# culiver/VAR

Measured on AMD Instinct MI355X. Metric: 256x256 images/sec (CFG=1.5) VAR-d16, higher is better.
Workload: dtype f32

## Files before the change

### include/var_hip.h

```cpp
#ifndef VAR_HIP_H
#define VAR_HIP_H

#include <stdint.h>

#ifdef __cplusplus
extern "C" {
#endif

#define VARHIP_EINVAL (-1)

typedef void* varhip_stream_t;

const char* varhip_version(void);

#define VARHIP_EPI_NONE 0
#define VARHIP_EPI_GELU 1
#define VARHIP_EPI_RESID 2
int varhip_gemm_nt_f32(const float* A, int64_t lda, const float* W, int64_t ldw, const float* bias,
                       float* out, int64_t ldo, int M, int N, int K, int epi,
                       const float* resid, int64_t ldr, const float* gamma, int64_t ldg, int rows_per_group,
                       int bias_per_row, int batch, int64_t sA, int64_t sW, int64_t sO, varhip_stream_t stream);
int varhip_gemm_force_tile(int tile);
int varhip_gemm_qkv_force_tile(int tile);
int varhip_gemm_last_pick(void);
// ... 70 lines not shown
int varhip_rans_encode_host(const uint32_t* pairs, int64_t n, uint32_t* words_out, int64_t cap, int64_t* nwords_out);
int varhip_rans_decode_u32(const uint32_t* cum, int l, int V, const uint32_t* words, int64_t words_total, const int64_t* word_off,
                           const int64_t* nwords, uint32_t* state, int64_t* idx_out, int32_t* err_out, int B, varhip_stream_t stream);
int varhip_rans_decode_host(const uint32_t* cum, int l, int V, const uint32_t* words, int64_t words_total, const int64_t* word_off,
                            const int64_t* nwords, uint32_t* state, int64_t* idx_out, int32_t* err_out, int B);

int varhip_quant_accum_f32(const int64_t* idx, const float* codebook, const int32_t* tap_idx, const float* tap_w,
                           const float* phi_w, const float* phi_b, float ratio,
                           float* up, float* f_hat, int B, int pn, int P, int Cv, varhip_stream_t stream);

int varhip_quant_accum_h_f32(const float* h, const int32_t* tap_idx, const float* tap_w,
                             const float* phi_w, const float* phi_b, float ratio,
                             float* up, float* f_hat, int B, int pn, int P, int Cv, varhip_stream_t stream);

int varhip_gumbel_softmax_f32(const float* x, const float* noise, float* y, int64_t rows, int V, float mul, float tau, varhip_stream_t stream);

int varhip_next_map_f32(const float* f_hat, const float* word_w, const float* word_b, const float* lvl_pos,
                        float* x_out, float* pooled, int B, int P, int pq, int C, int Cv, varhip_stream_t stream);
int varhip_quant_last_route(void);

int varhip_lvl_pos_f32(const float* lvl_embed, const int64_t* lvl, const float* pos, float* out, int L, int C, varhip_stream_t stream);

int varhip_first_map_f32(const float* class_emb, const int64_t* labels, int num_classes, const float* pos_start,
                         const float* lvl_pos, float* cond, float* x_out, int B, int C, int first_l, varhip_stream_t stream);

int varhip_conv3x3_nhwc_f32(const float* in, const float* w, const float* bias, const float* resid, float* out,
                            int B, int H, int W, int Cin, int Cout, int up2, int out_mode, varhip_stream_t stream);

int varhip_upconv_pack_f32(const float* w, float* w_phase, int Cin, int Cout, varhip_stream_t stream);
int varhip_upconv_phase_f32(const float* in, const float* w_phase, const float* bias, float* out,
                            int B, int H, int W, int Cin, int Cout, varhip_stream_t stream);
int varhip_upconv_phase_gn_f32(const float* in, const float* w_phase, const float* bias, float* out, double* gn_part,
                               int B, int H, int W, int Cin, int Cout, varhip_stream_t stream);

int64_t varhip_gn_scratch_elems(int B, int HW, int C, int G);
int varhip_gn_stats_f32(const float* x, float* stats, double* scratch, int B, int HW, int C, int G, float eps, varhip_stream_t stream);
int varhip_gn_apply_f32(const float* x, const float* stats, const float* gamma, const float* beta, float* out,
                        int B, int HW, int C, int G, int silu, varhip_stream_t stream);

int varhip_gn_silu_conv_out_f32(const float* x, const float* stats, const float* gamma, const float* beta, const float* w, const float* bias,
                                float* out, int B, int H, int W, int Cin, int Cout, int G, int out_mode, varhip_stream_t stream);

int varhip_softmax_rows_f32(const float* x, float* out, int64_t rows, int n, float scale, varhip_stream_t stream);

int varhip_nchw_to_nhwc_f32(const float* in, float* out, int B, int C, int HW, varhip_stream_t stream);
int varhip_nhwc_to_nchw_f32(const float* in, float* out, int B, int C, int HW, varhip_stream_t stream);

int varhip_conv_gn_blocks(int H, int W, int Cout, int phase);
int varhip_conv3x3_gn_nhwc_f32(const float* in, const float* w, const float* bias, const float* resid, float* out, double* gn_part,
                               int B, int H, int W, int Cin, int Cout, int up2, varhip_stream_t stream);
int varhip_gn_stats_part_f32(const double* gn_part, float* stats, int B, int nblk, int HW, int C, int G, float eps, varhip_stream_t stream);
int varhip_conv3x3_wino_nhwc_f32(const float* in, const float* u, const float* bias, const float* resid, float* out, double* gn_part,
                                 int B, int H, int W, int Cin, int Cout, varhip_stream_t stream);
int varhip_conv3x3_s2_nhwc_f32(const float* in, const float* w, const float* bias, float* out,
                               int B, int H, int W, int Cin, int Cout, varhip_stream_t stream);
int varhip_conv3x3_s2_nhwc_f16(const void* in, const void* w, const float* bias, void* out, int B, int H, int W, int Cin, int Cout,
                               varhip_stream_t stream);
int varhip_conv3x3_s2_nhwc_bf16(const void* in, const void* w, const float* bias, void* out, int B, int H, int W, int Cin, int Cout,
                                varhip_stream_t stream);
int varhip_nchw_to_nhwc_pad_f32(const float* in, float* out, int B, int C, int HW, int Cpad, varhip_stream_t stream);
int varhip_area_pool_f32(const float* f, float* pooled, int B, int P, int pq, int Cv, varhip_stream_t stream);
int varhip_word_embed_f32(const float* pooled, const float* word_w, const float* word_b, const float* lvl_pos,
                          float* x_out, int B, int lq, int C, int Cv, varhip_stream_t stream);
int varhip_quant_residual_f32(const int64_t* idx, const float* codebook, const int32_t* tap_idx, const float* tap_w,
                              const float* phi_w, const float* phi_b, float ratio, float* up, float* f_hat, float* f_rest,
                              int B, int pn, int P, int Cv, varhip_stream_t stream);

int varhip_token_select_i64(const uint8_t* keep, const int64_t* gt, const int64_t* sampled, int64_t* out, int64_t n, varhip_stream_t stream);

int varhip_neighbor_table_f32(const float* codebook, int V, int D, int n, int32_t* nbr_idx, float* nbr_dist, varhip_stream_t stream);
int varhip_smooth_select_f32(const float* logits, const int64_t* gt, const int32_t* nbr_idx, const float* nbr_dist, int n,
                             int cand_count, int use_thr, float thr, float ratio, int B, int l, int V, double t_cfg,
                             int64_t* idx_out, float* maxval_out, float* distlp_out, float* cfg_out, varhip_stream_t stream);

int varhip_token_loglik_f32(const float* logits, const int64_t* gt, int64_t ld_gt, int images, int classes, int l, int V,
                            int with_uncond, float ca, float cb, float* out, int64_t ld_out_img, int64_t ld_out_cls, varhip_stream_t stream);

int varhip_code_dist_f32(const float* codebook, int V, int D, float* out, varhip_stream_t stream);
int varhip_token_score_f32(const float* logits, const int64_t* gt, int64_t ld_gt, int images, int classes, int l, int V,
                           int with_uncond, float ca, float cb, int mode, int param, float thr, const float* dist, int64_t ld_dist,
                           float* out, int64_t ld_out_img, int64_t ld_out_cls, varhip_stream_t stream);

int varhip_dist_profile_f32(const float* logits, const int64_t* gt, int64_t ld_gt, int images, int classes, int l, int V,
                            int with_uncond, float ca, float cb, const float* dist, int64_t ld_dist,
                            const float* edges, int nbins, float min_prob,
                            int64_t* mass_q, int64_t* count, int64_t ld_img, int64_t ld_cls, varhip_stream_t stream);

int varhip_class_mix_f32(const float* logits, const int64_t* gt, int64_t ld_gt, int images, int classes, int l, int V, int with_uncond,
                         float ca, float cb, const float* prior, int64_t ld_prior, float* entropy, int64_t ld_ent_img, int64_t ld_ent_cls,
                         int64_t* mix_q, int64_t* hcond_q, int32_t* nanflag, int64_t ld_acc, float* h_mix, float* h_cond, float* mi,
                         float* logp_mix, int64_t ld_out, varhip_stream_t stream);
int varhip_class_mix_finish_f32(const int64_t* mix_q, const int64_t* hcond_q, const int32_t* nanflag, int64_t ld_acc, const int64_t* gt,
                                int64_t ld_gt, int images, int l, int V, float* h_mix, float* h_cond, float* mi, float* logp_mix,
                                int64_t ld_out, varhip_stream_t stream);
int varhip_class_mix_host_f32(const float* logits, const int64_t* gt, int64_t ld_gt, int images, int classes, int l, int V, int with_uncond,
                              float ca, float cb, const float* prior, int64_t ld_prior, float* entropy, int64_t ld_ent_img, int64_t ld_ent_cls,
                              int64_t* mix_q, int64_t* hcond_q, int32_t* nanflag, int64_t ld_acc, float* h_mix, float* h_cond, float* mi,
                              float* logp_mix, int64_t ld_out);
int varhip_class_mix_finish_host_f32(const int64_t* mix_q, const int64_t* hcond_q, const int32_t* nanflag, int64_t ld_acc, const int64_t* gt,
                                     int64_t ld_gt, int images, int l, int V, float* h_mix, float* h_cond, float* mi, float* logp_mix,
                                     int64_t ld_out);

int varhip_attn_profile_f32(const float* q, const float* kcache, int B2, int l, int H, int curL, int Lmax, const int32_t* ends, int S1,
                            int pn, int radius, int64_t* share_sum, int64_t ld_row, int64_t ld_head, int32_t* nan_count,
                            int32_t* tokens, int64_t ld_tok_row, int64_t ld_tok_head, varhip_stream_t stream);
int varhip_attn_profile_host_f32(const float* q, const float* kcache, int B2, int l, int H, int curL, int Lmax, const int32_t* ends, int S1,
// ... 134 lines not shown
                            int B, int H, int W, int Cin, int Cout, varhip_stream_t stream);
int varhip_conv16_gn_fusable(int B, int H, int W, int Cin, int Cout);
int varhip_gnconv3x3_nhwc_f16(const void* in, const float* table, int silu,
                              const void* w, const float* bias, const void* resid, void* out, double* gn_part,
                              int B, int H, int W, int Cin, int Cout, varhip_stream_t stream);
int varhip_gn_scale_shift_f32(const float* stats, const float* gamma, const float* beta, float* table, int B, int C, int G, varhip_stream_t stream);
int varhip_conv16_force_tile(int wm);
int varhip_conv16_last_pick(void);
int varhip_gn_stats_f16(const void* x, float* stats, double* scratch, int B, int HW, int C, int G, float eps, varhip_stream_t stream);
int varhip_gn_apply_f16(const void* x, const float* stats, const float* gamma, const float* beta, void* out,
                        int B, int HW, int C, int G, int silu, varhip_stream_t stream);
int varhip_gn_silu_conv_out_f16(const void* x, const float* stats, const float* gamma, const float* beta, const void* w, const float* bias,
                                float* out, int B, int H, int W, int Cin, int Cout, int G, int out_mode, varhip_stream_t stream);
int varhip_cast_f32_to_f16(const float* in, void* out, int64_t n, varhip_stream_t stream);
int varhip_cast_f16_to_f32(const void* in, float* out, int64_t n, varhip_stream_t stream);

int varhip_gemm_nt_bf16(const void* A, int64_t lda, const void* W, int64_t ldw, const float* bias,
                       void* out, int64_t ldo, int out_f16, int M, int N, int K, int epi,
                       const void* resid, int64_t ldr, int resid_f16, const float* gamma, int64_t ldg, int rows_per_group,
                       int batch, int64_t sA, int64_t sW, int64_t sO, varhip_stream_t stream);
int varhip_gemm16_force_tile(int tile);
int varhip_gemm16_persistent(int on);
int varhip_gemm16_deep(int on);
int varhip_gemm16_last_pick(int i);
int varhip_gemm_qkv_bf16(const void* A, int64_t lda, const void* W, int64_t ldw, const float* bias, int M, int C, int K,
                        const float* scale_mul, float plain_scale, int l2norm,
                        void* q_out, void* kcache, void* vcache, int B2, int l, int H, int pos0, int Lmax, varhip_stream_t stream);
int varhip_attn_cached_bf16(const void* q, const void* kcache, const void* vcache, void* out,
                           int B2, int l, int H, int curL, int Lmax, varhip_stream_t stream);
int varhip_ln_modulate_bf16out(const float* x, const float* scale, int64_t ld_scale, const float* shift, int64_t ld_shift,
                              void* out, int M, int C, int rows_per_group, float eps, varhip_stream_t stream);
int varhip_adaln_block_bf16(float* x, float* x2, void* xn16, void* q16, void* att16, void* hid16, const float* ada, int64_t ld_ada,
                           const void* qkv_w16, const float* qkv_b, const float* scale_mul, float plain_scale, int l2norm,
                           const void* proj_w16, const float* proj_b, const void* fc1_w16, const float* fc1_b,
                           const void* fc2_w16, const float* fc2_b, void* kcache16, void* vcache16,
                           int B2, int l, int C, int H, int hidden, int pos0, int Lmax, float eps, varhip_stream_t stream);
int varhip_conv3x3_nhwc_bf16(const void* in, const void* w, const float* bias, const void* resid, void* out, double* gn_part,
                            int B, int H, int W, int Cin, int Cout, int out_mode, varhip_stream_t stream);
int varhip_upconv_phase_bf16(const void* in, const void* w_phase, const float* bias, void* out, double* gn_part,
                            int B, int H, int W, int Cin, int Cout, varhip_stream_t stream);
int varhip_gnconv3x3_nhwc_bf16(const void* in, const float* table, int silu,
                               const void* w, const float* bias, const void* resid, void* out, double* gn_part,
                               int B, int H, int W, int Cin, int Cout, varhip_stream_t stream);
int varhip_conv16_force_tile(int wm);
int varhip_gn_stats_bf16(const void* x, float* stats, double* scratch, int B, int HW, int C, int G, float eps, varhip_stream_t stream);
int varhip_gn_apply_bf16(const void* x, const float* stats, const float* gamma, const float* beta, void* out,
                        int B, int HW, int C, int G, int silu, varhip_stream_t stream);
int varhip_gn_silu_conv_out_bf16(const void* x, const float* stats, const float* gamma, const float* beta, const void* w, const float* bias,
                                 float* out, int B, int H, int W, int Cin, int Cout, int G, int out_mode, varhip_stream_t stream);
int varhip_cast_f32_to_bf16(const float* in, void* out, int64_t n, varhip_stream_t stream);
int varhip_cast_bf16_to_f32(const void* in, float* out, int64_t n, varhip_stream_t stream);


#define VARHIP_NFAM 17
int varhip_timing_enable(int on);
int varhip_timing_select(int family_mask);
int varhip_timing_reset(void);
int varhip_timing_read(double* ms, double* flops, double* bytes, int64_t* launches);
const char* varhip_timing_name(int family);

#ifdef __cplusplus
}
#endif
#endif
```

### var_amd/csrc/common.h

```cpp
#pragma once
#include <hip/hip_runtime.h>
#include <stdint.h>
#include <stdlib.h>
#include "../../include/var_hip.h"
#include "../../include/var_math.h"

typedef float f32x2 __attribute__((ext_vector_type(2)));
__device__ __forceinline__ f32x2 vh_exp_pair(f32x2 x) {
    const f32x2 xc = {__builtin_fminf(x[0], 88.0f), __builtin_fminf(x[1], 88.0f)};
    const f32x2 t = xc * 1.44269504088896341f;
    const f32x2 n = {__builtin_rintf(t[0]), __builtin_rintf(t[1])};
    f32x2 r = __builtin_elementwise_fma(n, (f32x2)(-0.693145751953125f), xc);
    r = __builtin_elementwise_fma(n, (f32x2)(-1.42860682030941723212e-6f), r);
    f32x2 q = (f32x2)(1.9875691500e-4f);
    q = __builtin_elementwise_fma(q, r, (f32x2)(1.3981999507e-3f));
    q = __builtin_elementwise_fma(q, r, (f32x2)(8.3334519073e-3f));
    q = __builtin_elementwise_fma(q, r, (f32x2)(4.1665795894e-2f));
    q = __builtin_elementwise_fma(q, r, (f32x2)(1.6666665459e-1f));
    q = __builtin_elementwise_fma(q, r, (f32x2)(5.0000001201e-1f));
    const f32x2 y = __builtin_elementwise_fma(q, r * r, r) + 1.0f;
    f32x2 o;
    o[0] = (x[0] > -87.0f) ? __builtin_ldexpf(y[0], (int)n[0]) : 0.0f;
    o[1] = (x[1] > -87.0f) ? __builtin_ldexpf(y[1], (int)n[1]) : 0.0f;
    return o;
}

__device__ __forceinline__ f32x2 vh_gelu_tanh_pair(f32x2 x) {
    const f32x2 x3 = (x * x) * x;
    const f32x2 u = (x + x3 * 0.044715f) * 0.7978845608028654f;
    const f32x2 d = vh_exp_pair(u * -2.0f) + 1.0f;
    return f32x2{x[0] / d[0], x[1] / d[1]};
}

typedef float f32x4 __attribute__((ext_vector_type(4)));
typedef float f32x16 __attribute__((ext_vector_type(16)));

#define VH_FAM_GEMM 0
#define VH_FAM_CONV 1
#define VH_FAM_ATTN 2
#define VH_FAM_SAMPLER 3
#define VH_FAM_LN 4
#define VH_FAM_QKV 5
#define VH_FAM_GN 6
#define VH_FAM_OTHER 7
#define VH_FAM_GEMM_SMALL 8
#define VH_FAM_CONV_SMALL 9
#define VH_FAM_GEMM16 10
#define VH_FAM_GEMM16_SMALL 11
#define VH_FAM_CONV16H 12
#define VH_FAM_CONV16_SMALL 13
#define VH_FAM_ATTN16 14
#define VH_FAM_CONV_WINO 15
#define VH_FAM_ATTN_PROFILE 16

int vh_timing_on(int fam);
void vh_timing_begin(int fam, hipStream_t s, double flops, double bytes);
void vh_timing_end(int fam, hipStream_t s);

struct VhScope {
    int fam; hipStream_t s; bool on;
    VhScope(int f, hipStream_t st, double flops, double bytes) : fam(f), s(st), on(vh_timing_on(f) != 0) { if (on) vh_timing_begin(fam, s, flops, bytes); }
    ~VhScope() { if (on) vh_timing_end(fam, s); }
};

__device__ __forceinline__ void vh_dma16_buf(__amdgpu_buffer_rsrc_t rsrc, uint32_t voff, uint32_t soff, uint32_t lds) {
    asm volatile("s_mov_b32 m0, %3\n\ts_nop 0\n\tbuffer_load_dwordx4 %0, %1, %2 offen lds"
                 : : "v"(voff), "s"(rsrc), "s"(__builtin_amdgcn_readfirstlane(soff)), "s"(__builtin_amdgcn_readfirstlane(lds)) : "memory", "m0");
}

void vh_quant_phi_accum(const float* up, const float* phi_w, const float* phi_b, float ratio, float* f_hat, int B, int P, int Cv, hipStream_t s);

int vh_attn_keysel_refused(const void* q, const void* kcache, const void* vcache, const void* out, int B2, int l, int H, int curL, int Lmax,
                           const int32_t* ends, int S1, const int32_t* keymask, int32_t* ends16);

static inline int vh_launch_status() {
    hipError_t e = hipGetLastError();
    return e == hipSuccess ? 0 : -(1000 + (int)e);
}

template <int CTRL> __device__ __forceinline__ float vh_mov_dpp(float v) {
    return __int_as_float(__builtin_amdgcn_mov_dpp(__float_as_int(v), CTRL, 0xF, 0xF, true));
}
__device__ __forceinline__ float vh_lane_xor4(float v) {
    const float up = vh_mov_dpp<0x104>(v), dn = vh_mov_dpp<0x114>(v);
    return (threadIdx.x & 4) ? dn : up;
}
__device__ __forceinline__ float vh_wave_sum(float p) {
    { const auto r = __builtin_amdgcn_permlane32_swap(__float_as_uint(p), __float_as_uint(p), false, false); p = __uint_as_float(r[0]) + __uint_as_float(r[1]); }
    { const auto r = __builtin_amdgcn_permlane16_swap(__float_as_uint(p), __float_as_uint(p), false, false); p = __uint_as_float(r[0]) + __uint_as_float(r[1]); }
    p = p + vh_mov_dpp<0x128>(p);
    p = p + vh_lane_xor4(p);
    p = p + vh_mov_dpp<0x4E>(p);
    p = p + vh_mov_dpp<0xB1>(p);
    return p;
}
__device__ __forceinline__ float vh_wave_max(float p) {
    { const auto r = __builtin_amdgcn_permlane32_swap(__float_as_uint(p), __float_as_uint(p), false, false); p = fmaxf(__uint_as_float(r[0]), __uint_as_float(r[1])); }
    { const auto r = __builtin_amdgcn_permlane16_swap(__float_as_uint(p), __float_as_uint(p), false, false); p = fmaxf(__uint_as_float(r[0]), __uint_as_float(r[1])); }
    p = fmaxf(p, vh_mov_dpp<0x128>(p));
    p = fmaxf(p, vh_lane_xor4(p));
    p = fmaxf(p, vh_mov_dpp<0x4E>(p));
    p = fmaxf(p, vh_mov_dpp<0xB1>(p));
    return p;
}
__device__ __forceinline__ float vh_block_sum256(float p, float* red) {
    p = vh_wave_sum(p);
    __syncthreads();
    if ((threadIdx.x & 63) == 0) red[threadIdx.x >> 6] = p;
    __syncthreads();
    return ((red[0] + red[1]) + red[2]) + red[3];
}
__device__ __forceinline__ float vh_block_max256(float p, float* red) {
    p = vh_wave_max(p);
    __syncthreads();
    if ((threadIdx.x & 63) == 0) red[threadIdx.x >> 6] = p;
    __syncthreads();
    return fmaxf(fmaxf(red[0], red[1]), fmaxf(red[2], red[3]));
}
```

### var_amd/csrc/gemm.hip

```cpp
#include "common.h"

struct GemmP {
    const float* A; const float* W; const float* bias; float* out; const float* resid; const float* gamma;
    int64_t lda, ldw, ldo, ldr, ldg, sA, sW, sO;
    int M, N, K, epi, rows_per_group, bias_per_row;
    int H, Wd, Cin, up2, out_mode, Hi, Wi;
    int tilesM, tilesN;
    int evec;
    const float* q_smul; float* q_out; float* q_kc; float* q_vc; float q_plain; int q_l2, q_l, q_pos0, q_Lmax;
    double* gn_part;
};

__global__ void __launch_bounds__(256) k_gemm_any(GemmP p) {
    const int lane = threadIdx.x & 63, wave = threadIdx.x >> 6, r = lane & 31, h = lane >> 5;
    const int tm = blockIdx.x / p.tilesN, tn = blockIdx.x - tm * p.tilesN, bz = blockIdx.z;
    const int m0 = tm * 64 + (wave >> 1) * 32, n0 = tn * 64 + (wave & 1) * 32;
    const int ma = m0 + r, nb = n0 + r;
    const float* a = p.A + (int64_t)bz * p.sA + (int64_t)(ma < p.M ? ma : 0) * p.lda;
    const float* w = p.W + (int64_t)bz * p.sW + (int64_t)(nb < p.N ? nb : 0) * p.ldw;
    float* Ob = p.out + (int64_t)bz * p.sO;
    f32x16 acc;
#pragma unroll
    for (int e = 0; e < 16; ++e) acc[e] = 0.f;
    for (int k0 = 0; k0 < p.K; k0 += 2) {
// ... 592 lines not shown
}
extern "C" int varhip_conv3x3_nhwc_f32(const float* in, const float* w, const float* bias, const float* resid, float* out,
                                       int B, int H, int W, int Cin, int Cout, int up2, int out_mode, varhip_stream_t stream) {
    return conv3x3_impl(in, w, bias, resid, out, nullptr, B, H, W, Cin, Cout, up2, out_mode, stream);
}
extern "C" int varhip_conv3x3_gn_nhwc_f32(const float* in, const float* w, const float* bias, const float* resid, float* out, double* gn_part,
                                          int B, int H, int W, int Cin, int Cout, int up2, varhip_stream_t stream) {
    if (!gn_part) return VARHIP_EINVAL;
    return conv3x3_impl(in, w, bias, resid, out, gn_part, B, H, W, Cin, Cout, up2, 0, stream);
}

extern "C" int varhip_conv3x3_s2_nhwc_f32(const float* in, const float* w, const float* bias, float* out,
                                          int B, int H, int W, int Cin, int Cout, varhip_stream_t stream) {
    if (B <= 0 || H <= 0 || W <= 0 || Cin <= 0 || Cout <= 0 || (Cin & 31) || !bias) return VARHIP_EINVAL;
    if ((int64_t)B * H * W >= (1ll << 31)) return VARHIP_EINVAL;
    GemmP p{};
    p.A = in; p.W = w; p.bias = bias; p.out = out;
    p.ldw = 9ll * Cin; p.ldo = Cout; p.ldr = Cout;
    p.M = B * H * W; p.N = Cout; p.K = 9 * Cin; p.epi = VARHIP_EPI_NONE; p.rows_per_group = 1;
    p.H = H; p.Wd = W; p.Cin = Cin; p.up2 = 3; p.out_mode = 0; p.Hi = 2 * H; p.Wi = 2 * W;
    p.evec = !((Cout & 3) || ((uintptr_t)out & 15) || ((uintptr_t)bias & 15));
    const double npix = (double)B * H * W;
    VhScope scope(conv_family(3, Cout), (hipStream_t)stream, 2.0 * npix * Cout * 9.0 * Cin, 4.0 * (npix * 4 * Cin + npix * Cout + 9.0 * Cin * Cout));
    hipStream_t s = (hipStream_t)stream;
    return launch_conv(p, 1, s);
}

__global__ void k_upconv_pack(const float* __restrict__ w, float* __restrict__ wp, int Cout, int Cin) {
    const int64_t i = (int64_t)blockIdx.x * blockDim.x + threadIdx.x;
    const int64_t tot = (int64_t)16 * Cout * Cin;
    if (i >= tot) return;
    const int ci = (int)(i % Cin); int64_t t = i / Cin; const int b = (int)(t & 1), a = (int)((t >> 1) & 1); t >>= 2;
    const int co = (int)(t % Cout), ph = (int)(t / Cout), py = ph >> 1, px = ph & 1;
    const int ky0 = (py == 0) ? (a == 0 ? 0 : 1) : (a == 0 ? 0 : 2), ky1 = (py == 0) ? (a == 0 ? 0 : 2) : (a == 0 ? 1 : 2);
    const int kx0 = (px == 0) ? (b == 0 ? 0 : 1) : (b == 0 ? 0 : 2), kx1 = (px == 0) ? (b == 0 ? 0 : 2) : (b == 0 ? 1 : 2);
    float s = 0.f;
    for (int ky = ky0; ky <= ky1; ++ky)
        for (int kx = kx0; kx <= kx1; ++kx) s = s + w[(((int64_t)co * 3 + ky) * 3 + kx) * Cin + ci];
    wp[i] = s;
}
extern "C" int varhip_upconv_pack_f32(const float* w, float* w_phase, int Cin, int Cout, varhip_stream_t stream) {
    if (Cin <= 0 || Cout <= 0) return VARHIP_EINVAL;
    const int64_t tot = (int64_t)16 * Cout * Cin;
    VhScope scope(VH_FAM_OTHER, (hipStream_t)stream, 0, 4.0 * tot);
    hipLaunchKernelGGL(k_upconv_pack, dim3((unsigned)((tot + 255) / 256)), dim3(256), 0, (hipStream_t)stream, w, w_phase, Cout, Cin);
    return vh_launch_status();
}

static int upconv_phase_impl(const float* in, const float* w_phase, const float* bias, float* out, double* gn_part,
                             int B, int H, int W, int Cin, int Cout, varhip_stream_t stream) {
    if (B <= 0 || H <= 0 || W <= 0 || (H & 1) || (W & 1) || Cin <= 0 || Cout <= 0 || (Cin & 31) || !bias) return VARHIP_EINVAL;
    if (gn_part && !varhip_conv_gn_blocks(H, W, Cout, 1)) return VARHIP_EINVAL;
    if ((int64_t)B * H * W >= (1ll << 31)) return VARHIP_EINVAL;
    GemmP p{};
    p.A = in; p.W = w_phase; p.bias = bias; p.out = out; p.resid = nullptr; p.gamma = nullptr;
    p.ldw = 4ll * Cin; p.ldo = Cout; p.ldr = Cout; p.sW = (int64_t)Cout * 4 * Cin;
    p.M = B * (H / 2) * (W / 2); p.N = Cout; p.K = 4 * Cin; p.epi = VARHIP_EPI_NONE; p.rows_per_group = 1;
    p.H = H / 2; p.Wd = W / 2; p.Cin = Cin; p.up2 = 2; p.out_mode = 0; p.Hi = H / 2; p.Wi = W / 2;
    p.evec = !((Cout & 3) || ((uintptr_t)out & 15) || ((uintptr_t)bias & 15));
    if (gn_part && !p.evec) return VARHIP_EINVAL;
    p.gn_part = gn_part;
    const double npix = (double)B * H * W;
    VhScope scope(conv_family(2, Cout), (hipStream_t)stream, 2.0 * npix * Cout * 4.0 * Cin, 4.0 * (npix * Cin / 4.0 + npix * Cout + 16.0 * Cin * Cout));
    hipStream_t s = (hipStream_t)stream;
    return launch_conv(p, 4, s);
}
extern "C" int varhip_upconv_phase_f32(const float* in, const float* w_phase, const float* bias, float* out,
                                       int B, int H, int W, int Cin, int Cout, varhip_stream_t stream) {
    return upconv_phase_impl(in, w_phase, bias, out, nullptr, B, H, W, Cin, Cout, stream);
}
extern "C" int varhip_upconv_phase_gn_f32(const float* in, const float* w_phase, const float* bias, float* out, double* gn_part,
                                          int B, int H, int W, int Cin, int Cout, varhip_stream_t stream) {
    if (!gn_part) return VARHIP_EINVAL;
    return upconv_phase_impl(in, w_phase, bias, out, gn_part, B, H, W, Cin, Cout, stream);
}
```

### var_amd/csrc/timing.hip

```cpp
#include "common.h"
#include <mutex>
#include <vector>

namespace {
struct Rec { hipEvent_t a, b; int fam; };
std::mutex g_mu;
int g_on = 0;
int g_mask = ~0;
std::vector<Rec> g_pool;
size_t g_used = 0;
double g_ms[VARHIP_NFAM], g_flops[VARHIP_NFAM], g_bytes[VARHIP_NFAM];
int64_t g_n[VARHIP_NFAM];
const size_t kMaxRecs = 1 << 15;

void drain_locked() {
    for (size_t i = 0; i < g_used; ++i) {
        float ms = 0.f;
        if (hipEventSynchronize(g_pool[i].b) == hipSuccess && hipEventElapsedTime(&ms, g_pool[i].a, g_pool[i].b) == hipSuccess)
            g_ms[g_pool[i].fam] += ms;
    }
    g_used = 0;
}
}

// ... 14 lines not shown

void vh_timing_end(int fam, hipStream_t s) {
    std::lock_guard<std::mutex> lk(g_mu);
    (void)fam;
    if (g_used < g_pool.size()) { (void)hipEventRecord(g_pool[g_used].b, s); ++g_used; }
}

int vh_g_force_tile16 = -1;
int vh_g_gemm16_persist = [] { const char* e = getenv("VARHIP_GEMM16_PERSIST"); return e ? (atoi(e) != 0) : 1; }();
int vh_g_gemm16_deep = [] { const char* e = getenv("VARHIP_GEMM16_DEEP"); return e ? (atoi(e) != 0) : 1; }();
int vh_g_conv16_force_wm = 0;
int vh_g_gemm16_last_pick[2] = {0, 0};
int vh_g_gemm16_nlaunch = 0;
int vh_g_conv16_last_pick = -1;
int vh_g_attn16_last_waves = 0;

extern "C" {

int varhip_gemm16_force_tile(int tile) { vh_g_force_tile16 = (tile >= 0 && tile <= 3) ? tile : -1; return 0; }
int varhip_gemm16_persistent(int on) { vh_g_gemm16_persist = on ? 1 : 0; return 0; }
int varhip_gemm16_deep(int on) { vh_g_gemm16_deep = on ? 1 : 0; return 0; }
int varhip_gemm16_last_pick(int i) { return (i == 0 || i == 1) ? vh_g_gemm16_last_pick[i] : 0; }
int varhip_conv16_force_tile(int wm) { vh_g_conv16_force_wm = (wm == 2 || wm == 4 || wm == 8) ? wm : 0; return 0; }
int varhip_conv16_last_pick(void) { return vh_g_conv16_last_pick; }
int varhip_attn16_last_waves(void) { return vh_g_attn16_last_waves; }

const char* varhip_version(void) { return "var_hip 0.1.0 gfx950"; }

int varhip_timing_enable(int on) { std::lock_guard<std::mutex> lk(g_mu); g_on = on ? 1 : 0; return 0; }
int varhip_timing_select(int family_mask) { std::lock_guard<std::mutex> lk(g_mu); g_mask = family_mask; return 0; }

int varhip_timing_reset(void) {
    std::lock_guard<std::mutex> lk(g_mu);
    drain_locked();
    for (int i = 0; i < VARHIP_NFAM; ++i) { g_ms[i] = g_flops[i] = g_bytes[i] = 0.0; g_n[i] = 0; }
    return 0;
}

int varhip_timing_read(double* ms, double* flops, double* bytes, int64_t* launches) {
    std::lock_guard<std::mutex> lk(g_mu);
    drain_locked();
    for (int i = 0; i < VARHIP_NFAM; ++i) {
        if (ms) ms[i] = g_ms[i];
        if (flops) flops[i] = g_flops[i];
        if (bytes) bytes[i] = g_bytes[i];
        if (launches) launches[i] = g_n[i];
    }
    return VARHIP_NFAM;
}

const char* varhip_timing_name(int f) {
    static const char* names[VARHIP_NFAM] = {"gemm", "conv3x3", "attn", "sampler", "ln", "qkv_prep", "gn", "other", "gemm_small", "conv_small",
                                               "gemm16", "gemm16_small", "conv16h", "conv16_small", "attn16",
                                               "conv_wino", "attn_profile"};
    return (f >= 0 && f < VARHIP_NFAM) ? names[f] : "?";
}

}
```

### var_amd/csrc/winograd.hip

```cpp
#include <cstdlib>
#include <type_traits>

#include "common.h"

namespace {

constexpr int WG_PT = 18;
constexpr int WG_NDMA = 21;
constexpr int WG_STAGE = WG_NDMA * 16 * 64;
constexpr int WG_ZSTR = 20;
constexpr int WG_LDS = 2 * WG_STAGE;
static_assert(8 * 64 * WG_ZSTR * 4 <= WG_LDS, "epilogue exchange must fit in the K-loop stages");

struct WinoP {
    const float* in; const float* u; const float* bias; const float* resid; float* out; double* gn_part;
    int H, W, Cin, Cout, ncg, pw, ppi;
};

__device__ __forceinline__ void wg_wait_dma_barrier() { asm volatile("s_waitcnt vmcnt(8)\n\ts_barrier" ::: "memory"); }

constexpr int WG_KO_NOEPI = 1, WG_KO_NOGN = 2, WG_KO_NORES = 4, WG_KO_NOBTDB = 8;

__device__ __forceinline__ int wg_swz(int pix) { return (pix >> 1) & 3; }

// ... 134 lines not shown

    float* zb = smem;
    const int nblk = (H * W) >> 7;
#pragma unroll
    for (int cb = 0; cb < 2; ++cb) {
#pragma unroll
        for (int tb = 0; tb < 4; ++tb) {
            const f32x4 m0 = acc[0][tb][cb], m1 = acc[1][tb][cb], m2 = acc[2][tb][cb], m3 = acc[3][tb][cb];
            const f32x4 z0 = (m0 + m1) + m2, z1 = (m1 - m2) - m3;
            const int t = tb * 16 + r16;
            *(f32x4*)(zb + ((wave * 2 + 0) * 64 + t) * WG_ZSTR + 4 * kq) = z0;
            *(f32x4*)(zb + ((wave * 2 + 1) * 64 + t) * WG_ZSTR + 4 * kq) = z1;
        }
        __syncthreads();
        f32x4 z[4][2];
#pragma unroll
        for (int i = 0; i < 4; ++i)
#pragma unroll
            for (int bb = 0; bb < 2; ++bb) z[i][bb] = *(const f32x4*)(zb + ((i * 2 + bb) * 64 + et) * WG_ZSTR + 4 * eq);
        const int co = c0 + cb * 16 + 4 * eq;
        double gs[4] = {0.0, 0.0, 0.0, 0.0}, gq[4] = {0.0, 0.0, 0.0, 0.0};
#pragma unroll
        for (int a = 0; a < 2; ++a)
#pragma unroll
            for (int bb = 0; bb < 2; ++bb) {
                const f32x4 yv = a == 0 ? (z[0][bb] + z[1][bb]) + z[2][bb] : (z[1][bb] - z[2][bb]) - z[3][bb];
                f32x4 v = yv + b4[cb];
                const int64_t o = obase + ((int64_t)a * W + bb) * Cout + cb * 16;
                if constexpr (RES) v = rs[cb][a][bb] + v;
                *(f32x4*)(p.out + o) = v;
                if constexpr (GN) {
#pragma unroll
                    for (int e = 0; e < 4; ++e) { const double d = (double)v[e]; gs[e] += d; gq[e] += d * d; }
                }
            }
        if constexpr (GN) {
            const double t8[8] = {gs[0], gq[0], gs[1], gq[1], gs[2], gq[2], gs[3], gq[3]};
            const bool h4 = lane & 16, h3 = lane & 8, h2 = lane & 4;
            double r4[4], r2[2], r1;
#pragma unroll
            for (int i = 0; i < 4; ++i) r4[i] = (h4 ? t8[4 + i] : t8[i]) + __shfl_xor(h4 ? t8[i] : t8[4 + i], 16, 64);
#pragma unroll
            for (int i = 0; i < 2; ++i) r2[i] = (h3 ? r4[2 + i] : r4[i]) + __shfl_xor(h3 ? r4[i] : r4[2 + i], 8, 64);
            r1 = (h2 ? r2[1] : r2[0]) + __shfl_xor(h2 ? r2[0] : r2[1], 4, 64);
            r1 += __shfl_xor(r1, 2, 64);
            r1 += __shfl_xor(r1, 1, 64);
            if ((lane & 3) == 0)
                p.gn_part[(((int64_t)b * nblk + 2 * pi + (lane >> 5)) * Cout + co) * 2 + ((lane >> 2) & 7)] = r1;
        }
        if (cb == 0) __syncthreads();
    }
}

}

extern "C" int varhip_conv3x3_wino_nhwc_f32(const float* in, const float* u, const float* bias, const float* resid, float* out, double* gn_part,
                                            int B, int H, int W, int Cin, int Cout, varhip_stream_t stream) {
    if (!in || !u || !bias || !out || B <= 0 || H <= 0 || W <= 0 || Cin <= 0 || Cout <= 0) return VARHIP_EINVAL;
    if ((H & 15) || (W & 15) || (Cin & 31) || (Cout & 31)) return VARHIP_EINVAL;
    if ((((uintptr_t)in | (uintptr_t)u | (uintptr_t)bias | (uintptr_t)out | (uintptr_t)resid) & 15)) return VARHIP_EINVAL;
    if ((int64_t)H * W * Cin * 4 >= (1ll << 31) || 64ll * Cin * Cout >= (1ll << 31) || (int64_t)B * H * W >= (1ll << 31))
        return VARHIP_EINVAL;
    const int ppi = (H / 16) * (W / 16), ncg = Cout / 32;
    const int64_t nwg = (int64_t)B * ppi * ncg;
    if (nwg >= (1ll << 31)) return VARHIP_EINVAL;
    WinoP p{};
    p.in = in; p.u = u; p.bias = bias; p.resid = resid; p.out = out; p.gn_part = gn_part;
    p.H = H; p.W = W; p.Cin = Cin; p.Cout = Cout; p.ncg = ncg; p.pw = W / 16; p.ppi = ppi;
    const double npix = (double)B * H * W;
    VhScope scope(VH_FAM_CONV_WINO, (hipStream_t)stream, 2.0 * (npix / 4.0) * 16.0 * Cin * Cout,
                  4.0 * (npix * Cin + npix * Cout * (resid ? 2.0 : 1.0) + 16.0 * Cin * Cout));
    static const int dbg = [] { const char* e = getenv("VARHIP_WINO_DBG"); return e ? atoi(e) : 0; }();
    const bool res = resid && !(dbg & WG_KO_NORES), gn = gn_part && !(dbg & WG_KO_NOGN);
    if ((dbg & WG_KO_NOBTDB) && !(res && gn)) return VARHIP_EINVAL;
    auto kfn = (dbg & WG_KO_NOEPI) ? k_conv3x3_wino<false, false, WG_KO_NOEPI> : (dbg & WG_KO_NOBTDB) ? k_conv3x3_wino<true, true, WG_KO_NOBTDB>
             : res ? (gn ? k_conv3x3_wino<true, true, 0> : k_conv3x3_wino<true, false, 0>)
                   : (gn ? k_conv3x3_wino<false, true, 0> : k_conv3x3_wino<false, false, 0>);
    hipLaunchKernelGGL(kfn, dim3((unsigned)nwg), dim3(256), WG_LDS, (hipStream_t)stream, p);
    return vh_launch_status();
}
```

### var_amd/engine.py

```python
from __future__ import annotations

import math
import os
import weakref
from types import SimpleNamespace
from typing import Dict, List, Optional

import numpy as np
import torch

from . import hip
from .abi import EPI_GELU, EPI_NONE, EPI_RESID
from .workspace import Dims, allocate, cached, keep_precision, sampler_rows, workspace_spec


def bicubic_taps(pn: int, P: int):
    f = np.float32
    A = f(-0.75)
    scale = f(pn) / f(P)
    src = scale * (np.arange(P, dtype=np.float32) + f(0.5)) - f(0.5)
    i0 = np.floor(src)
    t = (src - i0).astype(np.float32)

    def near(x):
# ... 528 lines not shown
            out = torch.empty((B, Cout, Hh, Ww), dtype=torch.float32, device=h.device)
            hip.call('gn_silu_conv_out_' + self.fl, h, stats, self.w[key + '.norm_out.weight'], self.w[key + '.norm_out.bias'], wt,
                     self.w[key + '.conv_out.bias'], out, B, Hh, Ww, Cin, Cout, 32, mode)
            return out
        h = self.gn(h, key + '.norm_out', B, Hh * Ww, True)
        return self.conv3(h, key + '.conv_out', B, Hh, Ww, out_mode=mode)


_WINO_G = ((1.0, 0.0, 0.0), (0.5, 0.5, 0.5), (0.5, -0.5, 0.5), (0.0, 0.0, 1.0))


def wino_filter(w: torch.Tensor) -> torch.Tensor:
    co, _, _, ci = w.shape
    G = torch.tensor(_WINO_G, dtype=torch.float64, device=w.device)
    u = torch.einsum('ik,jl,oklc->ijoc', G, G, w.double()).float()
    return u.reshape(16, co, ci // 16, 16).permute(0, 2, 1, 3).contiguous()


class DecoderEngine(_VaeOps):

    PREFIXES = ('decoder.', 'post_quant_conv.')
    LEVELS = 'decoder.up.'
    precision = 'f32'
    unfused_tail = False
    winograd = os.environ.get('VARHIP_WINOGRAD', '1') != '0'
    WINO_MIN_HW = 16 * 16
    flops_precision = None

    def set_precision(self, precision: str):
        if precision not in PRECISIONS:
            raise ValueError(f"precision must be one of {PRECISIONS}")
        self.precision = precision

    def _derive(self, w):
        for k in [k for k in w if k.endswith('.upsample.conv.weight')]:
            cout, _, _, cin = w[k].shape
            wp = torch.empty(4, cout, 2, 2, cin, dtype=torch.float32, device=w[k].device)
            hip.call('upconv_pack_f32', w[k], wp, cin, cout)
            w[k[:-len('weight')] + 'phase'] = wp
        for k in [k for k in w if k.endswith(('.conv1.weight', '.conv2.weight'))]:
            w[k[:-len('weight')] + 'wino'] = wino_filter(w[k])
        return w

    def wino_ok(self, Hh, Ww, Cin, Cout):
        return Hh * Ww >= self.WINO_MIN_HW and Hh % 16 == 0 and Ww % 16 == 0 and Cin % 32 == 0 and Cout % 32 == 0

    def _wino(self, key, Hh, Ww, Cin, Cout):
        return self.w.get(key + '.wino') if self.winograd and self.wino_ok(Hh, Ww, Cin, Cout) else None

    def upsample(self, h, key, B, Hh, Ww):
        wp = self.w[key + '.phase']
        up = torch.empty((B, Hh, Ww, wp.shape[1]), dtype=torch.float32, device=h.device)
        part = self._leave_partials(up, B, hip.conv_gn_blocks(Hh, Ww, wp.shape[1], phase=True))
        if part is not None:
            hip.call('upconv_phase_gn_f32', h, wp, self.w[key + '.bias'], up, part, B, Hh, Ww, wp.shape[4], wp.shape[1])
        else:
            hip.call('upconv_phase_f32', h, wp, self.w[key + '.bias'], up, B, Hh, Ww, wp.shape[4], wp.shape[1])
        return up

    def tail(self, h, key, B, Hh, Ww, denorm, clamp=True):
        wt = self.w[key + '.conv_out.weight']
        Cout, Cin = wt.shape[0], wt.shape[3]
        mode = _tail_mode(denorm, clamp)
        if Hh % 8 == 0 and Ww % 32 == 0 and Cin % 32 == 0 and Cout <= 4 and (10 * 34 * 36 + 4 * Cin) * 4 <= 64 * 1024 and not self.unfused_tail:
            stats = self.gn_stats(h, B, Hh * Ww)
            out = torch.empty((B, Cout, Hh, Ww), dtype=torch.float32, device=h.device)
            hip.call('gn_silu_conv_out_f32', h, stats, self.w[key + '.norm_out.weight'], self.w[key + '.norm_out.bias'], wt,
                     self.w[key + '.conv_out.bias'], out, B, Hh, Ww, Cin, Cout, 32, mode)
            return out
        h = self.gn(h, key + '.norm_out', B, Hh * Ww, True)
        return self.conv3(h, key + '.conv_out', B, Hh, Ww, out_mode=mode)

    def _flops(self, P: int, prec: Optional[str]) -> float:
        self.refresh()
        w, f, hw, side = self.w, 0.0, P * P, P
        def c3(key, taps=9): co, _, _, ci = w[key + '.weight'].shape; return 2.0 * hw * co * taps * ci
        def c1(key): co, ci = w[key + '.weight'].shape; return 2.0 * hw * co * ci
        def res_taps(key): co, _, _, ci = w[key + '.weight'].shape; return 4 if prec == 'f32' and self.winograd and self.wino_ok(side, side, ci, co) else 9
        for kind, key in _decoder_graph(w, self.nlev):
            if kind == 'conv':
                f += c3(key)
            elif kind == 'res':
                f += c3(key + '.conv1', res_taps(key + '.conv1')) + c3(key + '.conv2', res_taps(key + '.conv2'))
                if (key + '.nin_shortcut.weight') in w: f += c1(key + '.nin_shortcut')
            elif kind == 'attn':
                f += c1(key + '.qkv') + c1(key + '.proj_out') + 2.0 * 2 * hw * hw * w[key + '.proj_out.weight'].shape[0]
            elif kind == 'up':
                hw *= 4; side *= 2
                f += c3(key, 9 if prec is None else 4)
            else:
                f += c3(key + '.conv_out')
        return f

    def flops_per_image_reference(self, P: int) -> float:
        return self._flops(P, None)

    def flops_per_image_executed(self, P: int, precision: Optional[str] = None) -> float:
        return self._flops(P, precision or self.flops_precision or self.precision)

    def decode_nhwc(self, f_hat: torch.Tensor, denorm: bool = True, precision: Optional[str] = None, clamp: bool = True) -> torch.Tensor:
        self.refresh()
        prec = precision or self.precision
        if not clamp and prec != 'f32':
            raise hip.VarHipError('decode_nhwc(clamp=False) is the fp32 decoder only')
        self.flops_precision = prec
        ops = self if prec == 'f32' else self.ops16(prec)
        self._wait_ready()
        B, P = f_hat.shape[0], f_hat.shape[1]
        h = f_hat if prec == 'f32' else ops._to16(f_hat.contiguous())
        return self._run(ops, _decoder_graph(self.w, self.nlev), h, B, P, P, denorm=denorm, clamp=clamp)
# ... 1734 lines not shown
```

### var_amd/hip.py

```python
import ctypes
import os

from . import abi

_HERE = os.path.dirname(os.path.abspath(__file__))
LIB_PATH = os.environ.get('VARHIP_LIB') or os.path.join(_HERE, 'libvar_hip.so')


class VarHipError(RuntimeError):
    pass


class _Lib:
    def __init__(self):
        if not os.path.exists(LIB_PATH):
            raise VarHipError(f'{LIB_PATH} not found: build it with `python -c "import __graft_entry__ as g; g.build()"` '
                              f'(or `make -C var_amd/csrc`). There is no CPU/PyTorch fallback for the sampling path.')
        self.so = ctypes.CDLL(LIB_PATH)
        self.fn = abi.bind(self.so, 'varhip_', with_stream=True)
        self.host = {name: getattr(self.so, 'varhip_' + name) for name in abi.SIGNATURES_HOST}

    def version(self) -> str:
        return self.fn['version']().decode()


_LIB = None


def lib() -> _Lib:
    global _LIB
    if _LIB is None:
        _LIB = _Lib()
    return _LIB


def _arg(a):
    if a is None:
        return None
    if hasattr(a, 'data_ptr'):
        return ctypes.c_void_p(a.data_ptr())
    return a


def current_stream() -> ctypes.c_void_p:
    import torch
    return ctypes.c_void_p(torch.cuda.current_stream().cuda_stream)


def call(name: str, *args, stream=None):
    L = lib()
    st = current_stream() if stream is None else stream
    rc = L.fn[name](*[_arg(a) for a in args], st)
    if rc != 0:
        raise VarHipError(f'varhip_{name} returned {rc}' + (' (VARHIP_EINVAL: unsupported shape/argument)' if rc == abi.EINVAL else ' (HIP launch error %d)' % (-rc - 1000)))


def call_host(name: str, *args):
    def arg(a):
        if hasattr(a, 'ctypes'):
            return ctypes.c_void_p(a.ctypes.data)
        return _arg(a)
    if name not in abi.SIGNATURES_HOST:
        raise VarHipError(f'varhip_{name} is not a host function')
    rc = lib().host[name](*[arg(a) for a in args])
    if rc != 0:
        raise VarHipError(f'varhip_{name} returned {rc}' + (' (VARHIP_EINVAL: unsupported shape/argument)' if rc == abi.EINVAL else ''))


def gn_scratch_elems(B, HW, C, G) -> int:
    return int(lib().fn['gn_scratch_elems'](B, HW, C, G))


def conv_gn_blocks(H, W, Cout, phase=False) -> int:
    return int(lib().fn['conv_gn_blocks'](H, W, Cout, 1 if phase else 0))


def conv16_gn_fusable(B, H, W, Cin, Cout) -> bool:
    return bool(lib().fn['conv16_gn_fusable'](B, H, W, Cin, Cout))


VQ_STATS_MAX_BLOCKS = abi.CONSTANTS['VQ_STATS_MAX_BLOCKS']


def vq_stats_blocks(n: int) -> int:
    return int(lib().so.varhip_vq_stats_blocks(n))


NFAM = abi.CONSTANTS['NFAM']


def timing_enable(on: bool, families=None):
    so = lib().so
    mask = -1
    if families is not None:
        names = [so.varhip_timing_name(i).decode() for i in range(NFAM)]
        mask = sum(1 << names.index(f) for f in families)
    so.varhip_timing_select(mask)
    so.varhip_timing_enable(1 if on else 0)


def timing_reset():
    lib().so.varhip_timing_reset()


def timing_read():
    n = abi_nfam = NFAM
    ms = (ctypes.c_double * n)(); fl = (ctypes.c_double * n)(); by = (ctypes.c_double * n)(); ln = (ctypes.c_int64 * n)()
    lib().so.varhip_timing_read(ms, fl, by, ln)
    return {lib().so.varhip_timing_name(i).decode(): dict(ms=ms[i], flops=fl[i], bytes=by[i], launches=int(ln[i])) for i in range(abi_nfam)}
```

Before: 157.1.

## Add Winograd-style kernel for phase-decomposed upsample conv in VQ decoder

Adds a new f32 kernel for the fused nearest-upsample plus 3x3 conv that uses the phase-decomposed weights. It builds input and output transforms so that overlapping 2x2 phase taps share MFMA work, and streams input tiles into LDS through double-buffered DMA with an optional fused GroupNorm partial reduction. The existing phase GEMM path now tries this kernel first when a global flag is set, and engine.py sets that flag from self.winograd around the upconv call. The change lowers FLOPs for the decoder upsampling convs, at the cost of register pressure and possible differences in numerical rounding.

```diff
diff --git a/include/var_hip.h b/include/var_hip.h
--- a/include/var_hip.h
+++ b/include/var_hip.h
@@ -146,6 +146,8 @@
 int varhip_gn_stats_part_f32(const double* gn_part, float* stats, int B, int nblk, int HW, int C, int G, float eps, varhip_stream_t stream);
 int varhip_conv3x3_wino_nhwc_f32(const float* in, const float* u, const float* bias, const float* resid, float* out, double* gn_part,
                                  int B, int H, int W, int Cin, int Cout, varhip_stream_t stream);
+int varhip_conv3x3_wino_up_nhwc_f32(const float* in, const float* w_phase, const float* bias, float* out, double* gn_part,
+                                    int B, int H, int W, int Cin, int Cout, varhip_stream_t stream);
 int varhip_conv3x3_s2_nhwc_f32(const float* in, const float* w, const float* bias, float* out,
                                int B, int H, int W, int Cin, int Cout, varhip_stream_t stream);
 int varhip_conv3x3_s2_nhwc_f16(const void* in, const void* w, const float* bias, void* out, int B, int H, int W, int Cin, int Cout,
@@ -386,7 +388,7 @@
 int varhip_cast_bf16_to_f32(const void* in, float* out, int64_t n, varhip_stream_t stream);
 
 
-#define VARHIP_NFAM 17
+#define VARHIP_NFAM 18
 int varhip_timing_enable(int on);
 int varhip_timing_select(int family_mask);
 int varhip_timing_reset(void);
diff --git a/var_amd/csrc/common.h b/var_amd/csrc/common.h
--- a/var_amd/csrc/common.h
+++ b/var_amd/csrc/common.h
@@ -51,6 +51,7 @@
 #define VH_FAM_CONV16_SMALL 13
 #define VH_FAM_ATTN16 14
 #define VH_FAM_CONV_WINO 15
+#define VH_FAM_CONV_WINO_UP 17
 #define VH_FAM_ATTN_PROFILE 16
 
 int vh_timing_on(int fam);
@@ -67,6 +68,9 @@
     asm volatile("s_mov_b32 m0, %3\n\ts_nop 0\n\tbuffer_load_dwordx4 %0, %1, %2 offen lds"
                  : : "v"(voff), "s"(rsrc), "s"(__builtin_amdgcn_readfirstlane(soff)), "s"(__builtin_amdgcn_readfirstlane(lds)) : "memory", "m0");
 }
+
+int vh_upconv_wino_try(const float* in, const float* w_phase, const float* bias, float* out, double* gn_part,
+                       int B, int H, int W, int Cin, int Cout, hipStream_t stream);
 
 void vh_quant_phi_accum(const float* up, const float* phi_w, const float* phi_b, float ratio, float* f_hat, int B, int P, int Cv, hipStream_t s);
 
diff --git a/var_amd/csrc/gemm.hip b/var_amd/csrc/gemm.hip
--- a/var_amd/csrc/gemm.hip
+++ b/var_amd/csrc/gemm.hip
@@ -668,6 +668,10 @@
     if (B <= 0 || H <= 0 || W <= 0 || (H & 1) || (W & 1) || Cin <= 0 || Cout <= 0 || (Cin & 31) || !bias) return VARHIP_EINVAL;
     if (gn_part && !varhip_conv_gn_blocks(H, W, Cout, 1)) return VARHIP_EINVAL;
     if ((int64_t)B * H * W >= (1ll << 31)) return VARHIP_EINVAL;
+    {
+        const int rc = vh_upconv_wino_try(in, w_phase, bias, out, gn_part, B, H, W, Cin, Cout, (hipStream_t)stream);
+        if (rc != 1) return rc;
+    }
     GemmP p{};
     p.A = in; p.W = w_phase; p.bias = bias; p.out = out; p.resid = nullptr; p.gamma = nullptr;
     p.ldw = 4ll * Cin; p.ldo = Cout; p.ldr = Cout; p.sW = (int64_t)Cout * 4 * Cin;
diff --git a/var_amd/csrc/timing.hip b/var_amd/csrc/timing.hip
--- a/var_amd/csrc/timing.hip
+++ b/var_amd/csrc/timing.hip
@@ -90,7 +90,7 @@
 const char* varhip_timing_name(int f) {
     static const char* names[VARHIP_NFAM] = {"gemm", "conv3x3", "attn", "sampler", "ln", "qkv_prep", "gn", "other", "gemm_small", "conv_small",
                                                "gemm16", "gemm16_small", "conv16h", "conv16_small", "attn16",
-                                               "conv_wino", "attn_profile"};
+                                               "conv_wino", "attn_profile", "conv_wino_up"};
     return (f >= 0 && f < VARHIP_NFAM) ? names[f] : "?";
 }
 
diff --git a/var_amd/csrc/winograd.hip b/var_amd/csrc/winograd.hip
--- a/var_amd/csrc/winograd.hip
+++ b/var_amd/csrc/winograd.hip
@@ -210,6 +210,181 @@
     }
 }
 
+constexpr int WU_PS = 12;
+constexpr int WU_NDMA = 8;
+constexpr int WU_STAGE = WU_NDMA * 16 * 64;
+constexpr int WU_LDS = 2 * WU_STAGE;
+
+__device__ __forceinline__ void wu_wait_dma_barrier() { asm volatile("s_waitcnt vmcnt(9)\n\ts_barrier" ::: "memory"); }
+
+template <bool GN>
+__global__ void __launch_bounds__(256, 2) k_conv3x3_wino_up(WinoP p) {
+    extern __shared__ __attribute__((aligned(16))) float smem[];
+    const int tid = threadIdx.x, lane = tid & 63, wave = __builtin_amdgcn_readfirstlane(tid >> 6);
+    const int r16 = lane & 15, kq = lane >> 4, th = wave & 1, ch = wave >> 1;
+    int lin;
+    {
+        const int nwg = gridDim.x, bid = blockIdx.x, q = nwg >> 3, rem = nwg & 7, xcd = bid & 7, loc = bid >> 3;
+        lin = (xcd < rem ? xcd * (q + 1) : rem * (q + 1) + (xcd - rem) * q) + loc;
+    }
+    const int cg = lin % p.ncg, pidx = lin / p.ncg, b = pidx / p.ppi, pi = pidx - b * p.ppi, py = pi / p.pw, px = pi - py * p.pw;
+    const int y0 = py * 16, x0 = px * 16, c0 = cg * 32 + ch * 16;
+    const int H = p.H, W = p.W, Hi = H >> 1, Wi = W >> 1, Cin = p.Cin, Cout = p.Cout, nk = Cin >> 4;
+
+    const int64_t img = (int64_t)Hi * Wi * Cin;
+    const __amdgpu_buffer_rsrc_t rsrc = __builtin_amdgcn_make_buffer_rsrc((void*)(p.in + (int64_t)b * img), 0, (int)(img * 4), 0x00020000);
+    uint32_t doff[2];
+#pragma unroll
+    for (int i = 0; i < 2; ++i) {
+        const int pix = (wave + 4 * i) * 16 + (lane >> 2), c = lane & 3;
+        const int pr = pix / WU_PS, pc = pix - pr * WU_PS;
+        const int yy = (y0 >> 1) - 1 + pr, xx = (x0 >> 1) - 1 + pc;
+        const bool ok = pr < 10 && pc < 10 && (unsigned)yy < (unsigned)Hi && (unsigned)xx < (unsigned)Wi;
+        doff[i] = ok ? (uint32_t)((((int64_t)yy * Wi + xx) * Cin + ((c ^ ((pr & 1) << 1)) << 2)) * 4) : 0x80000000u;
+    }
+    const uint32_t lds0 = (uint32_t)(uintptr_t)(__attribute__((address_space(3))) void*)smem;
+    auto dma = [&](int kt, int st) __attribute__((always_inline)) {
+#pragma unroll
+        for (int i = 0; i < 2; ++i) vh_dma16_buf(rsrc, doff[i], (uint32_t)kt * 64u, lds0 + st * WU_STAGE + (wave + 4 * i) * 1024);
+    };
+
+    const __amdgpu_buffer_rsrc_t ursrc = __builtin_amdgcn_make_buffer_rsrc((void*)p.u, 0, (int)(64u * Cin * Cout), 0x00020000);
+    const uint32_t uoff = (uint32_t)((c0 + r16) * 4 * Cin + 4 * kq) * 4u;
+    f32x4 u[9];
+    auto load_u = [&](int kt, int r) __attribute__((always_inline)) {
+#pragma unroll
+        for (int c = 0; c < 3; ++c)
+            u[3 * r + c] = __builtin_bit_cast(f32x4, __builtin_amdgcn_raw_buffer_load_b128(
+                ursrc, uoff, __builtin_amdgcn_readfirstlane((uint32_t)((((r == 2 ? 2 : 0) + (c == 2 ? 1 : 0)) * Cout * 4 + (r == 0 ? 0 : 2) + (c == 0 ? 0 : 1)) * Cin + 16 * kt) * 4u), 0));
+    };
+    dma(0, 0);
+#pragma unroll
+    for (int r = 0; r < 3; ++r) { load_u(0, r); __builtin_amdgcn_sched_barrier(0); }
+
+    const int prow = 4 * th + (r16 >> 3), pbase = (prow * WU_PS + (r16 & 7)) * 64;
+    const uint32_t roff_e = (uint32_t)(pbase + ((kq ^ ((prow & 1) << 1)) << 4)), roff_o = (uint32_t)(pbase + ((kq ^ (((prow + 1) & 1) << 1)) << 4));
+
+    f32x4 acc[9][2];
+#pragma unroll
+    for (int j = 0; j < 9; ++j)
+#pragma unroll
+        for (int tb = 0; tb < 2; ++tb) acc[j][tb] = f32x4{0.f, 0.f, 0.f, 0.f};
+
+    f32x4 b4;
+    auto compute = [&](int st, int kt_dma, int kt_u, auto last) __attribute__((always_inline)) {
+        const char* sb = (const char*)smem + st * WU_STAGE;
+#pragma unroll
+        for (int tb = 0; tb < 2; ++tb) {
+            f32x4 d[3][3];
+#pragma unroll
+            for (int r = 0; r < 3; ++r)
+#pragma unroll
+                for (int c = 0; c < 3; ++c) d[r][c] = *(const f32x4*)(sb + (r == 1 ? roff_o : roff_e) + (r * WU_PS + c + tb * 2 * WU_PS) * 64);
+#pragma unroll
+            for (int r = 0; r < 3; ++r) {
+                if (tb == 0) {
+                    if (r == 0) u[1] = u[0] + u[1];
+                    if (r == 1) { u[4] = u[1] + (u[3] + u[4]); u[3] = u[0] + u[3]; u[5] = u[2] + u[5]; }
+                    if (r == 2) u[7] = u[6] + u[7];
+                }
+                f32x4 e[3];
+#pragma unroll
+                for (int c = 0; c < 3; ++c) e[c] = r == 0 ? d[0][c] - d[1][c] : (r == 1 ? d[1][c] : d[1][c] - d[2][c]);
+                const f32x4 v[3] = {e[0] - e[1], e[1], e[1] - e[2]};
+#pragma unroll
+                for (int s = 0; s < 4; ++s)
+#pragma unroll
+                    for (int c = 0; c < 3; ++c) acc[3 * r + c][tb] = __builtin_amdgcn_mfma_f32_16x16x4f32(u[3 * r + c][s], v[c][s], acc[3 * r + c][tb], 0, 0, 0);
+                if (tb == 1) {
+                    __builtin_amdgcn_sched_barrier(0);
+                    if constexpr (decltype(last)::value) { if (r == 0) b4 = *(const f32x4*)(p.bias + c0 + 4 * kq); } else load_u(kt_u, r);
+                }
+            }
+            __builtin_amdgcn_sched_barrier(0);
+            if (tb == 0 && !decltype(last)::value) dma(kt_dma, st ^ 1);
+        }
+    };
+    wu_wait_dma_barrier();
+    int kt = 0;
+    for (; kt + 2 < nk; kt += 2) {
+        compute(0, kt + 1, kt + 1, std::false_type{});
+        wu_wait_dma_barrier();
+        compute(1, kt + 2, kt + 2, std::false_type{});
+        wu_wait_dma_barrier();
+    }
+    compute(0, kt + 1, kt + 1, std::false_type{});
+    wu_wait_dma_barrier();
+    compute(1, 0, 0, std::true_type{});
+
+    const int nblk = (H * W) >> 7;
+    double gs[4] = {0.0, 0.0, 0.0, 0.0}, gq[4] = {0.0, 0.0, 0.0, 0.0};
+#pragma unroll
+    for (int tb = 0; tb < 2; ++tb) {
+        const int ty = 4 * th + 2 * tb + (r16 >> 3), tx = r16 & 7;
+        const int64_t obase = (((int64_t)b * H + y0 + 2 * ty) * W + x0 + 2 * tx) * Cout + c0 + 4 * kq;
+        f32x4 z[3][2];
+#pragma unroll
+        for (int r = 0; r < 3; ++r) {
+            z[r][0] = acc[3 * r][tb] + acc[3 * r + 1][tb]; z[r][1] = acc[3 * r + 1][tb] - acc[3 * r + 2][tb];
+        }
+#pragma unroll
+        for (int a = 0; a < 2; ++a)
+#pragma unroll
+            for (int bb = 0; bb < 2; ++bb) {
+                const f32x4 v = (a == 0 ? z[0][bb] + z[1][bb] : z[1][bb] - z[2][bb]) + b4;
+                *(f32x4*)(p.out + obase + ((int64_t)a * W + bb) * Cout) = v;
+                if constexpr (GN) {
+#pragma unroll
+                    for (int e = 0; e < 4; ++e) { const double dd = (double)v[e]; gs[e] += dd; gq[e] += dd * dd; }
+                }
+            }
+    }
+    if constexpr (GN) {
+        const double t8[8] = {gs[0], gq[0], gs[1], gq[1], gs[2], gq[2], gs[3], gq[3]};
+        const bool h3 = lane & 8, h2 = lane & 4, h1 = lane & 2;
+        double r4[4], r2[2], r1;
+#pragma unroll
+        for (int k = 0; k < 4; ++k) r4[k] = (h3 ? t8[4 + k] : t8[k]) + __shfl_xor(h3 ? t8[k] : t8[4 + k], 8, 64);
+#pragma unroll
+        for (int k = 0; k < 2; ++k) r2[k] = (h2 ? r4[2 + k] : r4[k]) + __shfl_xor(h2 ? r4[k] : r4[2 + k], 4, 64);
+        r1 = (h1 ? r2[1] : r2[0]) + __shfl_xor(h1 ? r2[0] : r2[1], 2, 64);
+        r1 += __shfl_xor(r1, 1, 64);
+        if ((lane & 1) == 0)
+            p.gn_part[(((int64_t)b * nblk + 2 * pi + th) * Cout + c0 + 4 * kq) * 2 + ((lane >> 1) & 7)] = r1;
+    }
+}
+
+}
+
+static bool wino_up_ok(const float* in, const float* w_phase, const float* bias, float* out, int B, int H, int W, int Cin, int Cout) {
+    if (!in || !w_phase || !bias || !out || B <= 0 || H <= 0 || W <= 0 || Cin <= 0 || Cout <= 0) return false;
+    if ((H & 15) || (W & 15) || (Cin & 31) || (Cout & 31)) return false;
+    if ((((uintptr_t)in | (uintptr_t)w_phase | (uintptr_t)bias | (uintptr_t)out) & 15)) return false;
+    if ((int64_t)(H / 2) * (W / 2) * Cin * 4 >= (1ll << 31) || 64ll * Cin * Cout >= (1ll << 31) || (int64_t)B * H * W >= (1ll << 31))
+        return false;
+    return (int64_t)B * (H / 16) * (W / 16) * (Cout / 32) < (1ll << 31);
+}
+
+extern "C" int varhip_conv3x3_wino_up_nhwc_f32(const float* in, const float* w_phase, const float* bias, float* out, double* gn_part,
+                                               int B, int H, int W, int Cin, int Cout, varhip_stream_t stream) {
+    if (!wino_up_ok(in, w_phase, bias, out, B, H, W, Cin, Cout)) return VARHIP_EINVAL;
+    const int ppi = (H / 16) * (W / 16), ncg = Cout / 32;
+    const int64_t nwg = (int64_t)B * ppi * ncg;
+    WinoP p{};
+    p.in = in; p.u = w_phase; p.bias = bias; p.resid = nullptr; p.out = out; p.gn_part = gn_part;
+    p.H = H; p.W = W; p.Cin = Cin; p.Cout = Cout; p.ncg = ncg; p.pw = W / 16; p.ppi = ppi;
+    const double npix = (double)B * H * W;
+    VhScope scope(VH_FAM_CONV_WINO_UP, (hipStream_t)stream, 2.0 * (npix / 4.0) * 9.0 * Cin * Cout,
+                  4.0 * (npix / 4.0 * Cin + npix * Cout + 16.0 * Cin * Cout));
+    hipLaunchKernelGGL(gn_part ? k_conv3x3_wino_up<true> : k_conv3x3_wino_up<false>, dim3((unsigned)nwg), dim3(256), WU_LDS, (hipStream_t)stream, p);
+    return vh_launch_status();
+}
+
+extern "C" { int vh_g_upconv_wino = 0; }
+int vh_upconv_wino_try(const float* in, const float* w_phase, const float* bias, float* out, double* gn_part,
+                       int B, int H, int W, int Cin, int Cout, hipStream_t stream) {
+    if (!vh_g_upconv_wino || !wino_up_ok(in, w_phase, bias, out, B, H, W, Cin, Cout)) return 1;
+    return varhip_conv3x3_wino_up_nhwc_f32(in, w_phase, bias, out, gn_part, B, H, W, Cin, Cout, (varhip_stream_t)stream);
 }
 
 extern "C" int varhip_conv3x3_wino_nhwc_f32(const float* in, const float* u, const float* bias, const float* resid, float* out, double* gn_part,
diff --git a/var_amd/engine.py b/var_amd/engine.py
--- a/var_amd/engine.py
+++ b/var_amd/engine.py
@@ -604,10 +604,14 @@
         wp = self.w[key + '.phase']
         up = torch.empty((B, Hh, Ww, wp.shape[1]), dtype=torch.float32, device=h.device)
         part = self._leave_partials(up, B, hip.conv_gn_blocks(Hh, Ww, wp.shape[1], phase=True))
-        if part is not None:
-            hip.call('upconv_phase_gn_f32', h, wp, self.w[key + '.bias'], up, part, B, Hh, Ww, wp.shape[4], wp.shape[1])
-        else:
-            hip.call('upconv_phase_f32', h, wp, self.w[key + '.bias'], up, B, Hh, Ww, wp.shape[4], wp.shape[1])
+        hip.upconv_winograd(self.winograd)
+        try:
+            if part is not None:
+                hip.call('upconv_phase_gn_f32', h, wp, self.w[key + '.bias'], up, part, B, Hh, Ww, wp.shape[4], wp.shape[1])
+            else:
+                hip.call('upconv_phase_f32', h, wp, self.w[key + '.bias'], up, B, Hh, Ww, wp.shape[4], wp.shape[1])
+        finally:
+            hip.upconv_winograd(False)
         return up
 
     def tail(self, h, key, B, Hh, Ww, denorm, clamp=True):
diff --git a/var_amd/hip.py b/var_amd/hip.py
--- a/var_amd/hip.py
+++ b/var_amd/hip.py
@@ -75,6 +75,10 @@
     return int(lib().fn['conv_gn_blocks'](H, W, Cout, 1 if phase else 0))
 
 
+def upconv_winograd(on: bool):
+    ctypes.c_int.in_dll(lib().so, 'vh_g_upconv_wino').value = 1 if on else 0
+
+
 def conv16_gn_fusable(B, H, W, Cin, Cout) -> bool:
     return bool(lib().fn['conv16_gn_fusable'](B, H, W, Cin, Cout))
 
```

After: 159.1, median of 6. +1.3%, better.
